# NikolausDemmel/rootba

Measured on NVIDIA B200. Metric: ms/LM-iter (linearize+QR+PCG) on BAL at 1/2/4/8 B200 vs CPU ref, lower is better.
Workload: dtype f32

## Files before the change

rootba_b200/csrc/kernels.cuh:

```cuda
#pragma once

#include <cooperative_groups.h>
#include <cuda_runtime.h>

#include <cfloat>
#include <cmath>
#include <cstdint>

#include "layout.hpp"

namespace rba {

template <class S> struct ST;
template <> struct ST<float> {
  using V2 = float2;
  using V4 = float4;
  __host__ __device__ static float eps_sqrt() { return 0.0031622776601683794f; }
  __host__ __device__ static float eps() { return 1e-5f; }
  __host__ __device__ static float tiny() { return FLT_MIN; }
};
template <> struct ST<double> {
  using V2 = double2;
  using V4 = double4;
  __host__ __device__ static double eps_sqrt() { return 1e-5; }
// ... 1401 lines not shown
  for (int c = lane; c < CP; c += 32) {
    S v = 0;
    if (c < ncols) {
      const int i = c / 9, p = c - 9 * i;
      v = xvec[9 * (size_t)D.slot_cam[T.slot_base + i] + p];
    }
    xs[c] = v;
    ys[c] = 0;
  }
  __syncwarp();
  const V2* __restrict__ prow = reinterpret_cast<const V2*>(D.panel + T.panel_off) + (size_t)it.row0 * KP * 32 + lane;
  for (int r = 0; r < it.nrows; ++r) {
    S d = 0;
    for (int k = 0; k < KP; ++k) {
      const V2 v = __ldg(prow + (size_t)(r * KP + k) * 32);
      const int c = 2 * lane + 64 * k;
      d += v.x * xs[c] + v.y * xs[c + 1];
    }
    d = warp_sum(d);
    for (int k = 0; k < KP; ++k) {
      const V2 v = __ldg(prow + (size_t)(r * KP + k) * 32);
      const int c = 2 * lane + 64 * k;
      ys[c] += d * v.x;
      ys[c + 1] += d * v.y;
    }
  }
  __syncwarp();
  for (int c = lane; c < ncols; c += 32) D.yobs[9 * (size_t)it.yslot_base + c] = ys[c];
  __syncwarp();
}

__device__ __forceinline__ uint32_t smem_u32(const void* p) { return (uint32_t)__cvta_generic_to_shared(p); }
__device__ __forceinline__ void mbar_init(uint64_t* bar, uint32_t count) {
  asm volatile("mbarrier.init.shared::cta.b64 [%0], %1;" ::"r"(smem_u32(bar)), "r"(count) : "memory");
}
__device__ __forceinline__ void mbar_fence_init() {
  asm volatile("fence.mbarrier_init.release.cluster;" ::: "memory");
  asm volatile("fence.proxy.async.shared::cta;" ::: "memory");
}
__device__ __forceinline__ void mbar_expect_tx(uint64_t* bar, uint32_t bytes) {
  asm volatile("mbarrier.arrive.expect_tx.shared::cta.b64 _, [%0], %1;" ::"r"(smem_u32(bar)), "r"(bytes) : "memory");
}
__device__ __forceinline__ uint64_t l2_evict_first_policy() {
  uint64_t pol;
  asm volatile("createpolicy.fractional.L2::evict_first.b64 %0, 1.0;" : "=l"(pol));
  return pol;
}
__device__ __forceinline__ void bulk_g2s(void* dst, const void* src, uint32_t bytes, uint64_t* bar, uint64_t policy) {
  asm volatile("cp.async.bulk.shared::cluster.global.mbarrier::complete_tx::bytes.L2::cache_hint [%0], [%1], %2, [%3], %4;" ::"r"(
                   smem_u32(dst)),
               "l"(src), "r"(bytes), "r"(smem_u32(bar)), "l"(policy)
               : "memory");
}
__device__ __forceinline__ void mbar_wait(uint64_t* bar, uint32_t parity) {
  uint32_t ok;
  const uint32_t a = smem_u32(bar);
  do {
    asm volatile("{\n .reg .pred p;\n mbarrier.try_wait.parity.shared::cta.b64 p, [%1], %2;\n selp.u32 %0, 1, 0, p;\n}"
                 : "=r"(ok)
                 : "r"(a), "r"(parity)
                 : "memory");
  } while (!ok);
}

template <class S>
struct PanelStream {
  const S* src;
  int rows_left;
  int row_scalars;
  int rows_per_stage;
  int next_item;
  unsigned issued;
  uint64_t policy;
};

template <class S, int NS, int STAGE_BYTES>
__device__ __forceinline__ bool stream_produce(PanelStream<S>& ps, const DevPtrs<S>& D, const MatvecItem* __restrict__ items,
                                               int item_end, int item_stride, unsigned char* ring, uint64_t* bars, int lane) {
  if (ps.rows_left == 0) {
    if (ps.next_item >= item_end) return false;
    const MatvecItem it = items[ps.next_item];
    if (it.nrows == 0) { ps.next_item = item_end; return false; }
    const TileInfo T = D.tiles[it.tile];
    ps.row_scalars = T.KP * 64;
    ps.src = D.panel + T.panel_off + (size_t)it.row0 * ps.row_scalars;
    ps.rows_left = it.nrows;
    ps.rows_per_stage = max(1, STAGE_BYTES / (int)(ps.row_scalars * sizeof(S)));
    ps.next_item += item_stride;
  }
  const int rows = min(ps.rows_per_stage, ps.rows_left);
  const uint32_t bytes = (uint32_t)(rows * ps.row_scalars * sizeof(S));
  const unsigned slot = ps.issued % NS;
  if (lane == 0) {
    mbar_expect_tx(&bars[slot], bytes);
    bulk_g2s(ring + (size_t)slot * STAGE_BYTES, ps.src, bytes, &bars[slot], ps.policy);
  }
  ps.src += (size_t)rows * ps.row_scalars;
  ps.rows_left -= rows;
  ++ps.issued;
  return true;
}

template <class T>
__device__ __forceinline__ T group_sum_p(T v, int G) {
  T t;
  t = __shfl_xor_sync(0xffffffffu, v, 16); if (G > 16) v += t;
  t = __shfl_xor_sync(0xffffffffu, v, 8);  if (G > 8) v += t;
  t = __shfl_xor_sync(0xffffffffu, v, 4);  if (G > 4) v += t;
  t = __shfl_xor_sync(0xffffffffu, v, 2);  if (G > 2) v += t;
  t = __shfl_xor_sync(0xffffffffu, v, 1);  if (G > 1) v += t;
  return v;
}

template <class S, int KP, int NS, int STAGE_BYTES>
__device__ __forceinline__ void matvec_item_tma(const DevPtrs<S>& D, const MatvecItem& it, const TileInfo& T, int lane,
                                                const S* __restrict__ xvec, PanelStream<S>& ps, unsigned& consumed,
                                                const MatvecItem* __restrict__ items, int item_end, int item_stride,
                                                unsigned char* ring, uint64_t* bars) {
  using V2 = typename ST<S>::V2;
  const int n = T.n, G = T.G;
  const int g = lane / G, j = lane - g * G;
  const int ncols = 9 * n;
  const bool active = g < T.nvalid;
  const int slot0 = T.slot_base + g * n;
  int off0[KP], off1[KP];
  {
    const int step = 2 * G;
    const int di = step / 9, dp = step - 9 * di;
    int c = 2 * j;
    int i = c / 9, p = c - 9 * i;
#pragma unroll
    for (int k = 0; k < KP; ++k) {
      const bool v0 = active && c < ncols, v1 = active && (c + 1) < ncols;
      const int i1 = (p == 8) ? i + 1 : i, p1 = (p == 8) ? 0 : p + 1;
      const int cam0 = v0 ? __ldg(D.slot_cam + slot0 + i) : 0;
      const int cam1 = v1 ? __ldg(D.slot_cam + slot0 + i1) : 0;
      off0[k] = v0 ? 9 * cam0 + p : -1;
      off1[k] = v1 ? 9 * cam1 + p1 : -1;
      c += step; i += di; p += dp;
      if (p >= 9) { p -= 9; ++i; }
    }
  }
  V2 xv[KP], yv[KP];
#pragma unroll
  for (int k = 0; k < KP; ++k) {
    xv[k] = mk2(off0[k] >= 0 ? __ldg(xvec + off0[k]) : S(0), off1[k] >= 0 ? __ldg(xvec + off1[k]) : S(0));
    yv[k] = mk2(S(0), S(0));
  }
  int rows_left = it.nrows;
  constexpr int RPS = (STAGE_BYTES / (int)(KP * 64 * sizeof(S))) > 0 ? (STAGE_BYTES / (int)(KP * 64 * sizeof(S))) : 1;
  while (rows_left > 0) {
    const unsigned slot = consumed % NS;
    mbar_wait(&bars[slot], (consumed / NS) & 1u);
    const int rows = min(RPS, rows_left);
    const V2* st = reinterpret_cast<const V2*>(ring + (size_t)slot * STAGE_BYTES) + lane;
    int r = 0;
#ifndef RBA_K4_PAIR
#define RBA_K4_PAIR 0
#endif
    for (; RBA_K4_PAIR && r + 2 <= rows; r += 2) {
      V2 va[KP], vb[KP];
#pragma unroll
      for (int k = 0; k < KP; ++k) { va[k] = st[(r * KP + k) * 32]; vb[k] = st[((r + 1) * KP + k) * 32]; }
      S da0 = 0, da1 = 0, db0 = 0, db1 = 0;
#pragma unroll
      for (int k = 0; k < KP; ++k) {
        da0 = fma(va[k].x, xv[k].x, da0); da1 = fma(va[k].y, xv[k].y, da1);
        db0 = fma(vb[k].x, xv[k].x, db0); db1 = fma(vb[k].y, xv[k].y, db1);
      }
      S da = da0 + da1, db = db0 + db1;
      da = group_sum_p(da, G); db = group_sum_p(db, G);
#pragma unroll
      for (int k = 0; k < KP; ++k) {
        yv[k].x = fma(da, va[k].x, yv[k].x); yv[k].y = fma(da, va[k].y, yv[k].y);
        yv[k].x = fma(db, vb[k].x, yv[k].x); yv[k].y = fma(db, vb[k].y, yv[k].y);
      }
    }
    for (; r < rows; ++r) {
      V2 va[KP];
#pragma unroll
      for (int k = 0; k < KP; ++k) va[k] = st[(r * KP + k) * 32];
      S da0 = 0, da1 = 0;
#pragma unroll
      for (int k = 0; k < KP; ++k) { da0 = fma(va[k].x, xv[k].x, da0); da1 = fma(va[k].y, xv[k].y, da1); }
      S da = group_sum_p(da0 + da1, G);
#pragma unroll
      for (int k = 0; k < KP; ++k) { yv[k].x = fma(da, va[k].x, yv[k].x); yv[k].y = fma(da, va[k].y, yv[k].y); }
    }
    __syncwarp();
    ++consumed;
    rows_left -= rows;
    stream_produce<S, NS, STAGE_BYTES>(ps, D, items, item_end, item_stride, ring, bars, lane);
  }
  if (active) {
    S* yo = D.yobs + 9 * (size_t)(it.yslot_base + g * n);
#pragma unroll
    for (int k = 0; k < KP; ++k) {
      const int c = 2 * j + 2 * G * k;
      if (c < ncols) yo[c] = yv[k].x;
      if (c + 1 < ncols) yo[c + 1] = yv[k].y;
    }
  }
}

#ifndef RBA_K4_MINB
#define RBA_K4_MINB (sizeof(S) == 4 ? 5 : 2)
#endif
template <class S, int WARPS, int NS, int STAGE_BYTES>
__global__ void __launch_bounds__(WARPS * 32, RBA_K4_MINB) k_matvec_small_tma(DevPtrs<S> D, const MatvecItem* __restrict__ items,
                                                                  int item_begin, int item_end, int scratch_per_warp,
                                                                  const S* __restrict__ xvec, const int* done, int pdl) {
  extern __shared__ __align__(128) unsigned char smem_tma[];
  __shared__ __align__(8) uint64_t bars_all[WARPS][NS];
  if (done && *reinterpret_cast<const volatile int*>(done)) return;
  const int wib = threadIdx.x >> 5, lane = threadIdx.x & 31;
  unsigned char* ring = smem_tma + (size_t)wib * NS * STAGE_BYTES;
  uint64_t* bars = bars_all[wib];
  if (lane == 0) {
#pragma unroll
    for (int s = 0; s < NS; ++s) mbar_init(&bars[s], 1);
    mbar_fence_init();
  }
  __syncwarp();
  const int stride = gridDim.x * WARPS;
  const int first = item_begin + blockIdx.x * WARPS + wib;
  PanelStream<S> ps;
  ps.src = nullptr; ps.rows_left = 0; ps.row_scalars = 0; ps.rows_per_stage = 1; ps.next_item = first; ps.issued = 0; ps.policy = l2_evict_first_policy();
  unsigned consumed = 0;
#pragma unroll 1
  for (int s = 0; s < NS; ++s)
    if (!stream_produce<S, NS, STAGE_BYTES>(ps, D, items, item_end, stride, ring, bars, lane)) break;
  if (pdl) asm volatile("griddepcontrol.wait;" ::: "memory");
  if (done && *done) {
    for (unsigned s = 0; s < ps.issued; ++s) mbar_wait(&bars[s % NS], (s / NS) & 1u);
    return;
  }
  if (pdl) asm volatile("griddepcontrol.launch_dependents;" ::: "memory");
  for (int q = first; q < item_end; q += stride) {
    const MatvecItem it = items[q];
    if (it.nrows == 0) break;
    const TileInfo T = D.tiles[it.tile];
    switch (T.KP) {
      case 5: matvec_item_tma<S, 5, NS, STAGE_BYTES>(D, it, T, lane, xvec, ps, consumed, items, item_end, stride, ring, bars); break;
      case 6: matvec_item_tma<S, 6, NS, STAGE_BYTES>(D, it, T, lane, xvec, ps, consumed, items, item_end, stride, ring, bars); break;
      case 7: matvec_item_tma<S, 7, NS, STAGE_BYTES>(D, it, T, lane, xvec, ps, consumed, items, item_end, stride, ring, bars); break;
      case 8: matvec_item_tma<S, 8, NS, STAGE_BYTES>(D, it, T, lane, xvec, ps, consumed, items, item_end, stride, ring, bars); break;
      case 9: matvec_item_tma<S, 9, NS, STAGE_BYTES>(D, it, T, lane, xvec, ps, consumed, items, item_end, stride, ring, bars); break;
      default: break;
    }
  }
}

template <class S>
__device__ __forceinline__ void lds_rec28(const S* src, S (&v)[28]) {
  if (sizeof(S) == 4) {
    const float4* s4 = reinterpret_cast<const float4*>(src);
#pragma unroll
    for (int q = 0; q < 7; ++q) { const float4 t = s4[q]; v[4 * q] = t.x; v[4 * q + 1] = t.y; v[4 * q + 2] = t.z; v[4 * q + 3] = t.w; }
  } else {
    const double2* s2 = reinterpret_cast<const double2*>(src);
#pragma unroll
    for (int q = 0; q < 14; ++q) { const double2 t = s2[q]; v[2 * q] = t.x; v[2 * q + 1] = t.y; }
  }
}
template <class S>
__device__ __forceinline__ void lds_rec20(const S* src, S (&v)[20]) {
  if (sizeof(S) == 4) {
    const float4* s4 = reinterpret_cast<const float4*>(src);
#pragma unroll
    for (int q = 0; q < 5; ++q) { const float4 t = s4[q]; v[4 * q] = t.x; v[4 * q + 1] = t.y; v[4 * q + 2] = t.z; v[4 * q + 3] = t.w; }
  } else {
    const double2* s2 = reinterpret_cast<const double2*>(src);
#pragma unroll
    for (int q = 0; q < 10; ++q) { const double2 t = s2[q]; v[2 * q] = t.x; v[2 * q + 1] = t.y; }
  }
}

template <class S, int WARPS, int MAXSLOTS, int NS>
__global__ void __launch_bounds__(WARPS * 32) k_matvec_implicit_tma(DevPtrs<S> D, int tile_end, const S* __restrict__ xvec,
                                                                     const int* done, int pdl, int e0_only = 0) {
  static_assert(MAXSLOTS <= 64, "two observations per lane");
  extern __shared__ __align__(128) unsigned char smem_imp[];
  __shared__ __align__(8) uint64_t bars_all[WARPS][NS];
  if (done && *reinterpret_cast<const volatile int*>(done)) return;
  constexpr int QBYTES = MAXSLOTS * 28 * (int)sizeof(S), JBYTES = MAXSLOTS * 20 * (int)sizeof(S);
  constexpr int STAGE = QBYTES + JBYTES;
  const int wib = threadIdx.x >> 5, lane = threadIdx.x & 31;
  unsigned char* base = smem_imp + (size_t)wib * NS * STAGE;
  uint64_t* bars = bars_all[wib];
  if (lane == 0) {
#pragma unroll
    for (int s = 0; s < NS; ++s) mbar_init(&bars[s], 1);
    mbar_fence_init();
  }
  __syncwarp();
  const uint64_t policy = l2_evict_first_policy();
  const int stride = gridDim.x * WARPS;
  const int first = blockIdx.x * WARPS + wib;
  auto produce = [&](int t, int s) {
    if (lane == 0) {
// ... 667 lines not shown
```

rootba_b200/csrc/layout.hpp:

```cpp
#pragma once

#include <algorithm>
#include <cstdint>
#include <numeric>
#include <string>
#include <vector>

namespace rba {

struct TileInfo {
  long long panel_off;
  int slot_base;
  int lm_base;
  short n;
  short G;
  short KP;
  short nvalid;
};

struct MatvecItem {
  int tile;
  short row0, nrows;
  int yslot_base;
  int pad;
};

struct ReduceItem {
  int cam, begin, end;
};

struct CameraCSR {
  std::vector<int> cam_ptr;
  std::vector<int> slots;
  std::vector<ReduceItem> items;
  std::vector<int> cam_item_ptr;
};

struct Layout {
  int nc = 0;
  int lm_begin = 0, lm_end = 0;
  int nl_local = 0;
  long long nobs_local = 0;
  long long sum_n2 = 0;
  int max_n = 0;
  int kp_max = 0;
  std::vector<int> sorted_lm;
  std::vector<int> sorted_of_lm;
  std::vector<TileInfo> tiles;
  std::vector<int> tile_of_sorted;
  int nslots = 0;
  std::vector<int> slot_cam;
  std::vector<int> slot_lm;
  std::vector<long long> slot_obs;
  long long panel_scalars = 0;
  std::vector<MatvecItem> items;
  int n_items_large = 0;
  int nyslots = 0;
  CameraCSR csr_obs;
  CameraCSR csr_y;
  bool csr_y_is_obs = true;
  std::vector<ReduceItem> pb_items;
  std::vector<int> pb_cam_item_ptr;
  int k1_scratch_per_warp = 0;
  int k4_scratch_per_warp = 0;
};

constexpr int KP_SMALL_MAX = 9;
constexpr int ROWS_PER_ITEM = 32;
#ifndef RBA_SEG_LEN
#define RBA_SEG_LEN 96
#endif
constexpr int SEG_LEN = RBA_SEG_LEN;
constexpr int PB_SEG_LEN = 16;

inline int group_size_for(int n) {
  if (n <= 2) return 1;
  if (n <= 4) return 2;
// ... 77 lines not shown
  long long panel = 0;
  size_t pos = 0;
  while (pos < order.size()) {
    const int n = nloc[order[pos]];
    size_t end = pos;
    while (end < order.size() && nloc[order[end]] == n) ++end;
    const int G = group_size_for(n), W = 32 / G, KP = kp_for(n, G);
    for (size_t p = pos; p < end; p += W) {
      TileInfo T;
      T.panel_off = panel;
      T.slot_base = slot;
      T.lm_base = (int)L.sorted_lm.size();
      T.n = (short)n; T.G = (short)G; T.KP = (short)KP;
      T.nvalid = (short)std::min<size_t>(W, end - p);
      for (int g = 0; g < W; ++g) {
        const bool real = g < T.nvalid;
        const int lm = real ? order[p + g] : -1;
        if (real) L.sorted_of_lm[lm] = (int)L.sorted_lm.size();
        L.sorted_lm.push_back(lm);
        L.tile_of_sorted.push_back((int)L.tiles.size());
        for (int i = 0; i < n; ++i) {
          if (real) {
            const int64_t o = lm_off[L.lm_begin + lm] + i;
            L.slot_cam.push_back(obs_cam[o]);
            L.slot_lm.push_back(lm);
            L.slot_obs.push_back(o);
          } else {
            L.slot_cam.push_back(0);
            L.slot_lm.push_back(-1);
            L.slot_obs.push_back(-1);
          }
        }
      }
      slot += W * n;
      panel += (long long)2 * n * KP * 64;
      L.tiles.push_back(T);
    }
    pos = end;
  }
  L.nslots = slot;
  L.panel_scalars = panel;
  int extra = L.nslots;
  std::vector<int> ycam(L.slot_cam.size());
  for (int s = 0; s < L.nslots; ++s) ycam[s] = L.slot_lm[s] >= 0 ? L.slot_cam[s] : -1;
  for (int t = 0; t < (int)L.tiles.size(); ++t) {
    const TileInfo& T = L.tiles[t];
    const int rows = 2 * T.n, W = 32 / T.G;
    int nchunks = 1;
    if (rows > ROWS_PER_ITEM + ROWS_PER_ITEM / 2) nchunks = (rows + ROWS_PER_ITEM - 1) / ROWS_PER_ITEM;
    int r0 = 0;
    for (int c = 0; c < nchunks; ++c) {
      const int r1 = (int)((long long)rows * (c + 1) / nchunks);
      MatvecItem it;
      it.tile = t; it.row0 = (short)r0; it.nrows = (short)(r1 - r0); it.pad = 0;
      if (c == 0) {
        it.yslot_base = T.slot_base;
      } else {
        it.yslot_base = extra;
        for (int g = 0; g < W; ++g)
          for (int i = 0; i < T.n; ++i) {
            const int s = T.slot_base + g * T.n + i;
            ycam.push_back(L.slot_lm[s] >= 0 ? L.slot_cam[s] : -1);
          }
        extra += W * T.n;
        L.csr_y_is_obs = false;
      }
      L.items.push_back(it);
      r0 = r1;
    }
  }
  L.nyslots = extra;
  auto work = [&](const MatvecItem& it) {
    const TileInfo& T = L.tiles[it.tile];
    return (long long)it.nrows * T.KP;
  };
  std::stable_sort(L.items.begin(), L.items.end(), [&](const MatvecItem& a, const MatvecItem& b) {
    const bool la = L.tiles[a.tile].KP > KP_SMALL_MAX, lb = L.tiles[b.tile].KP > KP_SMALL_MAX;
    if (la != lb) return la;
    return work(a) > work(b);
  });
  L.n_items_large = 0;
  for (auto& it : L.items) if (L.tiles[it.tile].KP > KP_SMALL_MAX) ++L.n_items_large;
  {
    std::vector<int> ocam(ycam.begin(), ycam.begin() + L.nslots);
    build_csr(nc, L.nslots, ocam, L.csr_obs);
    if (!L.csr_y_is_obs) build_csr(nc, L.nyslots, ycam, L.csr_y);
    L.pb_cam_item_ptr.assign(nc + 1, 0);
    for (int c = 0; c < nc; ++c) {
      L.pb_cam_item_ptr[c] = (int)L.pb_items.size();
      for (int b = L.csr_obs.cam_ptr[c]; b < L.csr_obs.cam_ptr[c + 1]; b += PB_SEG_LEN)
        L.pb_items.push_back({c, b, std::min(b + PB_SEG_LEN, L.csr_obs.cam_ptr[c + 1])});
    }
    L.pb_cam_item_ptr[nc] = (int)L.pb_items.size();
  }
  for (const TileInfo& T : L.tiles) {
    const int W = 32 / T.G;
    L.k1_scratch_per_warp = std::max(L.k1_scratch_per_warp, W * 32 * (int)T.n);
    const int CS = (2 * T.G * T.KP) | 1;
    L.k4_scratch_per_warp = std::max(L.k4_scratch_per_warp, T.KP > kp_max ? 2 * 64 * (int)T.KP : W * CS);
  }
  return "";
}

}
```

rootba_b200/csrc/solver.cu:

```cuda
#include <cuda_runtime.h>
#include <dlfcn.h>

#include <cstdio>
#include <cstdlib>
#include <cstring>
#include <chrono>
#include <limits>
#include <memory>
#include <string>
#include <vector>

#include "../../include/rootba_b200.h"
#include "../host/bal_io_fast.hpp"
#include "kernels.cuh"
#include "nccl_dyn.hpp"

namespace rba {

thread_local std::string g_err;

#define CU(call)                                                                                   \
  do {                                                                                             \
    cudaError_t e__ = (call);                                                                      \
    if (e__ != cudaSuccess) {                                                                      \
// ... 11 lines not shown

using namespace rba;

struct rba_handle {
  int scalar_size = 0;
  virtual ~rba_handle() {}
  virtual int set_state(const void* cams, const void* lms) = 0;
  virtual int get_state(void* cams, void* lms) = 0;
  virtual int backup() = 0;
  virtual int restore() = 0;
  virtual int compute_error(rba_residual_info* out) = 0;
  virtual int linearize() = 0;
  virtual int solve(double lambda, void* inc_out, rba_cg_summary* cg) = 0;
  virtual int apply(const void* inc, void* l_diff_out, bool update_cameras) = 0;
  virtual int lm_step(bool linearize_first, double lambda, rba_lm_step_result* out) = 0;
  virtual int lm_run(const rba_lm_opts* o, int max_steps, rba_lm_iteration* log, int* steps_done, int* terminated, rba_stage_timings* totals) = 0;
  virtual int get_timings(rba_stage_timings* out) const = 0;
  virtual int get_stats(rba_workload_stats* out) const = 0;
  virtual int get_scaling(void* scaling, void* diag2) = 0;
  virtual int get_rhs(void* b) = 0;
  virtual int get_precond(void* inv, void* blocks) = 0;
  virtual int right_multiply(const void* x, void* y) = 0;
  virtual int debug_get_block(int lm, void* out, int rows, int cols, void* jls) = 0;
  virtual int time_matvec(int reps, double* sec) = 0;
  virtual int timer_start() = 0;
  virtual int timer_stop(double* sec) = 0;
  virtual void* stream_ptr() = 0;
  virtual int synchronize() = 0;
  virtual int comm_init(const void* uid) = 0;
  virtual int ipc_export(void* out128) = 0;
  virtual int ipc_import(const void* all) = 0;
};

#ifndef RBA_IMP_NS
#define RBA_IMP_NS 1
#endif

namespace rba {

template <class S>
struct Solver : rba_handle {
  rba_solver_opts opt{};
  KOpts ko{};
  Layout L;
  int nc = 0, nl_total = 0;
  int device = 0;
  int sm_count = 148;
  cudaStream_t stream = nullptr;
  std::vector<void*> allocs;
  size_t device_bytes = 0;
  DevPtrs<S> D{};
  S* cams_bk = nullptr; S* lms_bk = nullptr;
  MatvecItem* d_items = nullptr;
  std::vector<MatvecItem> dealt_items;
  int n_dealt = 0, dealt_grid = 0, dealt_bps = 0;
  long long state_version = 0;
  rba_residual_info error_cache{}; long long error_cache_version = -1, error_enqueue_version = -1; bool error_cache_valid = false;
  int* d_csr_obs_slots = nullptr; ReduceItem* d_csr_obs_items = nullptr; int* d_csr_obs_item_ptr = nullptr;
  int* d_csr_y_slots = nullptr; ReduceItem* d_csr_y_items = nullptr; int* d_csr_y_item_ptr = nullptr;
  int n_obs_items = 0, n_y_items = 0;
  const int* op_slots = nullptr; const ReduceItem* op_items = nullptr; const int* op_item_ptr = nullptr; int n_op_items = 0;
  bool implicit_op = false;
  int e0_only_flag = 0;
  bool panel_form = true;
  int imp_tile_split = 0;
  size_t imp_smem = 0; int imp_grid = 1;
  ReduceItem* d_pb_items = nullptr; int* d_pb_item_ptr = nullptr; int n_pb_items = 0;
  int pcg_cluster = 16;
  bool use_pdl = true;
  int* h_prog = nullptr; int* d_prog = nullptr;
  int pcg_solve_id = 0;
  bool pcg_partials = true;
  double* d_epart = nullptr;
  double* d_red = nullptr;
  int* d_flags = nullptr;
  int* d_cam_cnt = nullptr;
  PcgState* d_state = nullptr;
  PcgState* h_state = nullptr;
  double* h_red = nullptr;
  int* h_flags = nullptr;
  cudaEvent_t poll_ev[2] = {nullptr, nullptr};
  bool linearized = false;
  bool new_linearization_point = false;
  bool have_inc = false;
  S last_lambda = 0;
  bool damping_valid = false;
  rba_stage_timings tm{};
  EventPair ev_stage1, ev_stage2, ev_precond, ev_pcg, ev_backsub, ev_update, ev_error, ev_mv, ev_user;
  long long launches = 0;
  NcclApi* nccl = nullptr;
  ncclComm_t comm = nullptr;
  char* peer_mem = nullptr;
  size_t peer_bytes = 0;
  PeerComm pc{};
  bool peer_ok = false;
  int ar_seq = 0, c_seq = 0, s_seq = 0;
  std::vector<void*> ipc_opened;
  static constexpr int EBLOCKS = 592;
  static constexpr int KPMAX = sizeof(S) == 4 ? 16 : 10;

  ~Solver() override {
    if (comm && nccl) nccl->CommDestroy(comm);
    for (void* p : ipc_opened) cudaIpcCloseMemHandle(p);
    for (void* p : allocs) cudaFree(p);
    if (h_prog) cudaFreeHost(h_prog);
    if (h_state) cudaFreeHost(h_state);
// ... 61 lines not shown
    ko.use_valid_projections_only = opt.use_valid_projections_only;
    ko.robust_norm = opt.robust_norm;
    ko.write_panel = (opt.operator_form == 1 || opt.solver_type != 0) ? 0 : 1;
    ko.huber = opt.huber_parameter;
    ko.jacobi_eps = opt.jacobi_scaling_epsilon > 0 ? opt.jacobi_scaling_epsilon : (double)ST<S>::eps_sqrt();
    std::string msg = build_layout(nc, nl_total, pv->lm_obs_offset, pv->obs_cam_idx, opt.rank, opt.nranks, KPMAX, L);
    if (!msg.empty()) { g_err = msg; return RBA_ERR_INVALID_ARGUMENT; }
    std::vector<S> xy((size_t)2 * L.nslots, S(0));
    const S* src = (const S*)pv->obs_xy;
    for (int s = 0; s < L.nslots; ++s)
      if (L.slot_obs[s] >= 0) { xy[2 * (size_t)s] = src[2 * L.slot_obs[s]]; xy[2 * (size_t)s + 1] = src[2 * L.slot_obs[s] + 1]; }
    int rc;
    TileInfo* d_tiles; int* d_sorted; int* d_slot_cam; int* d_slot_lm; S* d_xy;
#define TRY(x) do { rc = (x); if (rc) return rc; } while (0)
    TRY(upload(&d_tiles, L.tiles));
    TRY(upload(&d_sorted, L.sorted_lm));
    TRY(upload(&d_slot_cam, L.slot_cam));
    TRY(upload(&d_slot_lm, L.slot_lm));
    TRY(upload(&d_xy, xy));
    dealt_items = L.items;
    n_dealt = (int)L.items.size();
    {
      const char* e = getenv("RBA_MATVEC_DEAL");
      long long deal_ovh = 48;
      if (const char* o2 = getenv("RBA_MATVEC_DEAL_OVH")) deal_ovh = atoll(o2);
      const int nsmall = (int)L.items.size() - L.n_items_large;
      int tma_bps = std::max(1, (int)((220 * 1024) / ((size_t)K4_WARPS * K4_NS * K4_STAGE + 1024)));
      {
        const size_t smem = (size_t)K4_WARPS * K4_NS * K4_STAGE;
        int occ = 0;
        if (cudaFuncSetAttribute((k_matvec_small_tma<S, K4_WARPS, K4_NS, K4_STAGE>), cudaFuncAttributeMaxDynamicSharedMemorySize, (int)smem) == cudaSuccess &&
            cudaOccupancyMaxActiveBlocksPerMultiprocessor(&occ, (k_matvec_small_tma<S, K4_WARPS, K4_NS, K4_STAGE>), K4_WARPS * 32, smem) == cudaSuccess && occ > 0)
          tma_bps = std::min(tma_bps, occ);
        else
          cudaGetLastError();
      }
      dealt_bps = tma_bps;
      const int W = grid_for(nsmall, K4_WARPS, tma_bps) * K4_WARPS;
      if (!(e && std::string(e) == "rr") && nsmall > W && !implicit_op) {
        std::vector<std::vector<int>> lists(W);
        std::vector<std::pair<long long, int>> heap(W);
        for (int w = 0; w < W; ++w) heap[w] = {0, w};
        auto cmp = [](const std::pair<long long, int>& a, const std::pair<long long, int>& b) { return a > b; };
        std::make_heap(heap.begin(), heap.end(), cmp);
        for (int q = L.n_items_large; q < (int)L.items.size(); ++q) {
          std::pop_heap(heap.begin(), heap.end(), cmp);
          auto& top = heap.back();
          lists[top.second].push_back(q);
          top.first += (long long)L.items[q].nrows * L.tiles[L.items[q].tile].KP + deal_ovh;
          std::push_heap(heap.begin(), heap.end(), cmp);
        }
        size_t maxlen = 0;
        for (auto& l : lists) maxlen = std::max(maxlen, l.size());
        MatvecItem empty{}; empty.tile = 0; empty.row0 = 0; empty.nrows = 0; empty.yslot_base = 0; empty.pad = 0;
        dealt_items.assign(L.items.begin(), L.items.begin() + L.n_items_large);
        dealt_items.resize(L.n_items_large + maxlen * W, empty);
        for (int w = 0; w < W; ++w)
          for (size_t k = 0; k < lists[w].size(); ++k) dealt_items[L.n_items_large + k * W + w] = L.items[lists[w][k]];
        n_dealt = (int)dealt_items.size();
        dealt_grid = W / K4_WARPS;
      }
    }
    TRY(upload(&d_items, dealt_items));

    TRY(upload(&d_csr_obs_slots, L.csr_obs.slots));
    TRY(upload(&d_csr_obs_items, L.csr_obs.items));
    TRY(upload(&d_csr_obs_item_ptr, L.csr_obs.cam_item_ptr));
    n_obs_items = (int)L.csr_obs.items.size();
    if (L.csr_y_is_obs) {
      d_csr_y_slots = d_csr_obs_slots; d_csr_y_items = d_csr_obs_items; d_csr_y_item_ptr = d_csr_obs_item_ptr;
      n_y_items = n_obs_items;
    } else {
      TRY(upload(&d_csr_y_slots, L.csr_y.slots));
      TRY(upload(&d_csr_y_items, L.csr_y.items));
      TRY(upload(&d_csr_y_item_ptr, L.csr_y.cam_item_ptr));
      n_y_items = (int)L.csr_y.items.size();
    }
    implicit_op = opt.operator_form == 1 || opt.solver_type != 0;
    if (opt.operator_form != 0 && opt.operator_form != 1) { g_err = "operator_form must be 0 (dense) or 1 (implicit)"; return RBA_ERR_INVALID_ARGUMENT; }
    if (opt.solver_type < 0 || opt.solver_type > 2) { g_err = "solver_type must be 0 (SQUARE_ROOT), 1 (SCHUR_COMPLEMENT) or 2 (POWER_SCHUR_COMPLEMENT)"; return RBA_ERR_INVALID_ARGUMENT; }
    if (opt.solver_type == 2 && opt.nranks > 1) { g_err = "POWER_SCHUR_COMPLEMENT runs on one GPU (the power-series vector kernel has no peer exchange yet)"; return RBA_ERR_UNSUPPORTED; }
    if (opt.power_order <= 0) opt.power_order = 20;
    if (opt.solver_type != 0) implicit_op = true;
    if (opt.stage2_form != 0 && opt.stage2_form != 1) { g_err = "stage2_form must be 0 (Q2 panel, reference) or 1 (orthogonality identity)"; return RBA_ERR_INVALID_ARGUMENT; }
    panel_form = !implicit_op && opt.stage2_form == 0;
    if (implicit_op) {
      while (imp_tile_split < (int)L.tiles.size() && (32 / L.tiles[imp_tile_split].G) * L.tiles[imp_tile_split].n <= IMP_MAXSLOTS) ++imp_tile_split;
      imp_smem = (size_t)IMP_WARPS * IMP_NS * (size_t)IMP_MAXSLOTS * 48 * sizeof(S);
      CU(cudaFuncSetAttribute((k_matvec_implicit_tma<S, IMP_WARPS, IMP_MAXSLOTS, IMP_NS>), cudaFuncAttributeMaxDynamicSharedMemorySize, (int)imp_smem));
      int bps = 0;
      CU(cudaOccupancyMaxActiveBlocksPerMultiprocessor(&bps, (k_matvec_implicit_tma<S, IMP_WARPS, IMP_MAXSLOTS, IMP_NS>), IMP_WARPS * 32, imp_smem));
      imp_grid = std::max(1, std::min((imp_tile_split + IMP_WARPS - 1) / IMP_WARPS, sm_count * std::max(1, bps)));
    }
    if (implicit_op) { op_slots = d_csr_obs_slots; op_items = d_csr_obs_items; op_item_ptr = d_csr_obs_item_ptr; n_op_items = n_obs_items; }
    else { op_slots = d_csr_y_slots; op_items = d_csr_y_items; op_item_ptr = d_csr_y_item_ptr; n_op_items = n_y_items; }
    TRY(upload(&d_pb_items, L.pb_items));
    TRY(upload(&d_pb_item_ptr, L.pb_cam_item_ptr));
    n_pb_items = (int)L.pb_items.size();
    D.tiles = d_tiles; D.ntiles = (int)L.tiles.size(); D.sorted_lm = d_sorted;
    D.slot_cam = d_slot_cam; D.slot_lm = d_slot_lm; D.slot_xy = d_xy; D.nslots = L.nslots; D.nc = nc;
    TRY(dalloc(&D.cams, (size_t)10 * nc)); TRY(dalloc(&cams_bk, (size_t)10 * nc));
    TRY(dalloc(&D.lms, (size_t)3 * L.nl_local)); TRY(dalloc(&lms_bk, (size_t)3 * L.nl_local));
    if (ko.write_panel) TRY(dalloc(&D.panel, (size_t)L.panel_scalars));
    TRY(dalloc(&D.jp, (size_t)20 * L.nslots));
    TRY(dalloc(&D.q1u, (size_t)28 * L.nslots));
    TRY(dalloc(&D.q1d, (size_t)28 * L.nslots));
    TRY(dalloc(&D.jl, (size_t)6 * L.nslots));
    TRY(dalloc(&D.res, (size_t)2 * L.nslots));
    TRY(dalloc(&D.lmk, (size_t)24 * L.sorted_lm.size()));
    TRY(dalloc(&D.qtr, (size_t)2 * L.nslots));
    if (panel_form) {
      TRY(dalloc(&D.dmp, (size_t)28 * L.nslots));
      if (opt.preconditioner_type == 1) TRY(dalloc(&D.blk0, (size_t)48 * L.nslots));
      TRY(dalloc(&D.blocks0, (size_t)81 * nc));
// ... 48 lines not shown
      };
      TRY(setup(k1_sc, K1_CAP, need1, k1_smem, k1_bps, k1_max_blocks));
      TRY(setup(k2_sc, K2_CAP, need2, k2_smem, k2_bps, k2_max_blocks));
      if (!(getenv("RBA_TILE_DEAL") && std::string(getenv("RBA_TILE_DEAL")) == "rr")) {
        TRY(deal_tiles(tile_grid(k1_max_blocks) * TILE_WARPS, order_k1));
        TRY(deal_tiles(tile_grid(sm_count * 8) * TILE_WARPS, order_kp));
      }
      CU(cudaFuncSetAttribute((k_linearize_qr<S, false>), cudaFuncAttributeMaxDynamicSharedMemorySize, (int)k1_smem));
      CU(cudaFuncSetAttribute((k_linearize_qr<S, true>), cudaFuncAttributeMaxDynamicSharedMemorySize, (int)k1_smem));
      CU(cudaFuncSetAttribute((k_stage2<S, true>), cudaFuncAttributeMaxDynamicSharedMemorySize, (int)k2_smem));
      CU(cudaFuncSetAttribute((k_stage2<S, false>), cudaFuncAttributeMaxDynamicSharedMemorySize, (int)k2_smem));
    }
    k4_smem_small = (size_t)K4_WARPS * L.k4_scratch_per_warp * sizeof(S);
    if (k4_smem_small > 200 * 1024) { g_err = "matvec scratch exceeds shared memory"; return RBA_ERR_UNSUPPORTED; }
    CU(cudaFuncSetAttribute(k_matvec_small<S, K4_WARPS>, cudaFuncAttributeMaxDynamicSharedMemorySize, (int)std::max<size_t>(k4_smem_small, 1024)));
    CU(cudaFuncSetAttribute((k_matvec_large<S, K4_WARPS, KPMAX>), cudaFuncAttributeMaxDynamicSharedMemorySize, (int)std::max<size_t>(k4_smem_small, 1024)));
    {
      CU(cudaFuncSetAttribute(k_pcg_vec<S>, cudaFuncAttributeNonPortableClusterSizeAllowed, 1));
      CU(cudaFuncSetAttribute(k_power_vec<S>, cudaFuncAttributeNonPortableClusterSizeAllowed, 1));
      pcg_cluster = 16;
      if (const char* e = getenv("RBA_PDL")) use_pdl = atoi(e) != 0;
      if (const char* e = getenv("RBA_PCG_PARTIALS")) pcg_partials = atoi(e) != 0;
      if (const char* e = getenv("RBA_PCG_CLUSTER")) pcg_cluster = std::max(1, std::min(atoi(e), 16));
      for (; pcg_cluster > 1; pcg_cluster >>= 1) {
        cudaLaunchConfig_t cfg = {};
        cfg.gridDim = dim3(pcg_cluster); cfg.blockDim = dim3(VEC_THREADS);
        cudaLaunchAttribute at[1];
        at[0].id = cudaLaunchAttributeClusterDimension;
        at[0].val.clusterDim.x = pcg_cluster; at[0].val.clusterDim.y = 1; at[0].val.clusterDim.z = 1;
        cfg.attrs = at; cfg.numAttrs = 1;
        int ncl = 0;
        if (cudaOccupancyMaxActiveClusters(&ncl, k_pcg_vec<S>, &cfg) == cudaSuccess && ncl >= 1) break;
        cudaGetLastError();
      }
    }
    {
      const char* e = getenv("RBA_MATVEC");
      use_tma = !(e && std::string(e) == "ldg");
      k4_smem_tma = (size_t)K4_WARPS * K4_NS * K4_STAGE;
      if (k4_smem_tma > 220 * 1024) use_tma = false;
      if (use_tma) {
        CU(cudaFuncSetAttribute((k_matvec_small_tma<S, K4_WARPS, K4_NS, K4_STAGE>), cudaFuncAttributeMaxDynamicSharedMemorySize, (int)k4_smem_tma));
        k4_tma_blocks_per_sm = std::max(1, (int)((220 * 1024) / (k4_smem_tma + 1024)));
        if (dealt_bps > 0) k4_tma_blocks_per_sm = dealt_bps;
        if (const char* b = getenv("RBA_MATVEC_BLOCKS_PER_SM")) k4_tma_blocks_per_sm = std::max(1, atoi(b));
      }
    }
#undef TRY
    CU(cudaStreamSynchronize(stream));
    return RBA_OK;
  }
  static constexpr int K4_WARPS = 4;
  static constexpr int IMP_WARPS = 2, IMP_MAXSLOTS = 64, IMP_NS = RBA_IMP_NS;
#ifndef RBA_K4_NS
#define RBA_K4_NS 2
#endif
#ifndef RBA_K4_STAGE
#define RBA_K4_STAGE 4608
#endif
  static constexpr int K4_NS = RBA_K4_NS;
  static constexpr int K4_STAGE = RBA_K4_STAGE;
  static constexpr int TILE_WARPS = 4;
  static constexpr int K1_CAP = 3904;
  static constexpr int K2_CAP = 3072;
  Scratch<S> k1_sc{}, k2_sc{};
  size_t k1_smem = 0, k2_smem = 0;
  int k1_bps = 2, k2_bps = 2, k1_max_blocks = 296, k2_max_blocks = 296;
  size_t k4_smem_small = 0, k4_smem_tma = 0;
  bool use_tma = true;
  int k4_tma_blocks_per_sm = 2;

  int allreduce(S* buf, size_t count) {
    if (opt.nranks == 1) return RBA_OK;
    if (peer_ok && (long long)count <= pc.cmax) {
      ++c_seq;
      const int g = (int)std::max<size_t>(1, std::min<size_t>((size_t)sm_count, (count + 255) / 256));
      k_peer_push<S><<<g, 256, 0, stream>>>(pc, buf, (long long)count, c_seq & 1);
      k_peer_sum<S><<<g, 256, 0, stream>>>(pc, buf, (long long)count, c_seq & 1, c_seq, d_flags + 1);
      launches += 2;
      return RBA_OK;
    }
    if (!comm) { g_err = "rba_comm_init has not been called on a sharded handle"; return RBA_ERR_STATE; }
    ncclResult_t r = nccl->AllReduce(buf, buf, count, sizeof(S) == 4 ? ncclFloat : ncclDouble, ncclSum, comm, stream);
    if (r != ncclSuccess) { g_err = std::string("ncclAllReduce: ") + nccl->GetErrorString(r); return RBA_ERR_NCCL; }
    return RBA_OK;
  }
  int allreduce_scalars(int nd) {
    if (opt.nranks == 1) return RBA_OK;
    if (peer_ok) {
      ++s_seq;
      k_peer_small<<<1, 64, 0, stream>>>(pc, d_red, nd, d_flags, 4, s_seq & 1, s_seq, d_flags + 1);
      ++launches;
      return RBA_OK;
    }
    if (!comm) { g_err = "rba_comm_init has not been called on a sharded handle"; return RBA_ERR_STATE; }
    ncclResult_t r = ncclSuccess;
    if (nd > 0) r = nccl->AllReduce(d_red, d_red, nd, ncclDouble, ncclSum, comm, stream);
    if (r == ncclSuccess) r = nccl->AllReduce(d_flags, d_flags, 4, ncclInt, ncclSum, comm, stream);
    if (r != ncclSuccess) { g_err = std::string("ncclAllReduce: ") + nccl->GetErrorString(r); return RBA_ERR_NCCL; }
    return RBA_OK;
  }

  int comm_init(const void* uid) override {
    if (opt.nranks == 1) return RBA_OK;
    nccl = nccl_api();
    if (!nccl) { g_err = "libnccl.so.2 could not be loaded"; return RBA_ERR_NCCL; }
    ncclUniqueId id;
    std::memcpy(&id, uid, sizeof(id));
    CU(cudaSetDevice(device));
    ncclResult_t r = nccl->CommInitRank(&comm, opt.nranks, id, opt.rank);
    if (r != ncclSuccess) { g_err = std::string("ncclCommInitRank: ") + nccl->GetErrorString(r); return RBA_ERR_NCCL; }
    return RBA_OK;
  }

// ... 190 lines not shown
    CU(cudaGetLastError());
    tm.stage1_time = elapsed(ev_stage1);
    tm.kernel_launches = launches - lin_l0;
    if (h_flags[4 + 1]) { linearized = false; g_err = "a peer rank did not take part in a cross-shard reduction in time (peer-memory exchange timed out)"; return RBA_ERR_NCCL; }
    if (h_flags[4 + 0]) { linearized = false; return RBA_NUMERICAL_FAILURE; }
    return RBA_OK;
  }
  int linearize() override {
    int rc = linearize_enqueue(); if (rc) return rc;
    CU(cudaStreamSynchronize(stream));
    return linearize_finish();
  }

  int precond_blocks(int mode, S* dst, const S* addend, bool reduce_ranks) {
    const int g = (n_pb_items + 127) / 128;
    switch (mode) {
      case 0: k_precond_partial<S, 0><<<g, 128, 0, stream>>>(D.jp, (const S*)nullptr, d_csr_obs_slots, d_pb_items, n_pb_items, D.pblk); break;
      case 1: k_precond_partial<S, 1><<<g, 128, 0, stream>>>(D.jp, D.q1d, d_csr_obs_slots, d_pb_items, n_pb_items, D.pblk); break;
      case 2: k_precond_partial<S, 2><<<g, 128, 0, stream>>>(D.dmp, (const S*)nullptr, d_csr_obs_slots, d_pb_items, n_pb_items, D.pblk); break;
      default: k_precond_partial<S, 3><<<g, 128, 0, stream>>>(D.blk0, (const S*)nullptr, d_csr_obs_slots, d_pb_items, n_pb_items, D.pblk); break;
    }
    k_precond_final<S><<<(45 * nc + 255) / 256, 256, 0, stream>>>(D.pblk, d_pb_item_ptr, nc, addend, dst);
    launches += 2;
    return reduce_ranks ? allreduce(dst, (size_t)81 * nc) : RBA_OK;
  }

  void matvec_launch(const S* xvec, const int* done) {
    matvec_kernels(xvec, done);
    k_cam_reduce_final<S, false><<<grid_for(n_op_items, 8, 8), 256, 0, stream>>>((const S*)D.yobs, op_slots, op_items, n_op_items, op_item_ptr, D.partial,
                                                                               d_cam_cnt, D.y, done, 0, pc, 0, nc);
    ++launches;
  }
  void matvec_kernels(const S* xvec, const int* done, bool pdl = false) {
    if (implicit_op) {
      const int ntl = (int)L.tiles.size();
      const bool p = pdl && use_pdl && imp_tile_split == ntl;
      if (imp_tile_split > 0 && use_tma)
        launch_ex((k_matvec_implicit_tma<S, IMP_WARPS, IMP_MAXSLOTS, IMP_NS>), imp_grid, IMP_WARPS * 32, imp_smem, p, 1, D, imp_tile_split, xvec, done, (int)p, e0_only_flag);
      const int tb = use_tma ? imp_tile_split : 0;
      if (tb < ntl)
        launch_ex(k_matvec_implicit<S>, (ntl - tb + TILE_WARPS - 1) / TILE_WARPS, TILE_WARPS * 32, 0, false, 1, D, tb, xvec, done, 0, e0_only_flag);
      ++tm.matvec_launches;
      return;
    }
    const int nitems = n_dealt;
    if (L.n_items_large > 0) {
      k_matvec_large<S, K4_WARPS, KPMAX><<<grid_for(L.n_items_large, K4_WARPS, 4), K4_WARPS * 32, k4_smem_small, stream>>>(
          D, d_items, 0, L.n_items_large, L.k4_scratch_per_warp, xvec, done);
      ++launches;
    }
    if (nitems > L.n_items_large) {
      if (use_tma) {
        launch_ex(k_matvec_small_tma<S, K4_WARPS, K4_NS, K4_STAGE>, dealt_grid > 0 ? dealt_grid : grid_for(nitems - L.n_items_large, K4_WARPS, k4_tma_blocks_per_sm), K4_WARPS * 32,
                  k4_smem_tma, pdl && use_pdl && L.n_items_large == 0, 1, D, (const MatvecItem*)d_items, L.n_items_large, nitems, L.k4_scratch_per_warp, xvec, done,
                  (int)(pdl && use_pdl && L.n_items_large == 0));
        --launches;
      } else
        k_matvec_small<S, K4_WARPS><<<grid_for(nitems - L.n_items_large, K4_WARPS, 5), K4_WARPS * 32, k4_smem_small, stream>>>(
            D, d_items, L.n_items_large, nitems, L.k4_scratch_per_warp, xvec, done);
      ++launches;
    }
    ++tm.matvec_launches;
  }
  int pcg_vec(int i, int mode, bool pdl, int is_last, S lambda, bool fused_ar = false, bool from_partials = false) {
    PeerComm c = pc;
    if (!fused_ar) c.nranks = 1;
    return launch_ex(k_pcg_vec<S>, pcg_cluster, VEC_THREADS, 0, pdl && use_pdl, pcg_cluster, D, d_state, lambda, i, mode, (double)opt.eta,
                     (int)opt.min_linear_solver_iterations, is_last, (int)(pdl && use_pdl), c, ar_seq, from_partials ? op_item_ptr : (const int*)nullptr, d_prog);
  }
  bool pcg_from_partials() const {
    return opt.nranks == 1 && pcg_partials && 9 * ((nc + pcg_cluster - 1) / pcg_cluster) <= VEC_THREADS * VEC_EPT;
  }
  int pcg_apply(int i, int mode, int is_last, S lambda) {
    if (pcg_from_partials()) {
      int rc = launch_ex(k_cam_reduce<S>, grid_for(n_op_items, 8, 8), 256, 0, use_pdl, 1, (const S*)D.yobs, op_slots, op_items, n_op_items, D.partial,
                         (const int*)&d_state->done, (int)use_pdl);
      if (rc) return rc;
      return pcg_vec(i, mode, true, is_last, lambda, false, true);
    }
    const bool fused = opt.nranks > 1 && peer_ok;
    if (fused) ++ar_seq;
    if (opt.nranks > 1 && !fused) CU(cudaMemsetAsync(D.y, 0, (size_t)9 * nc * sizeof(S), stream));
    int rc = fused ? launch_ex((k_cam_reduce_final<S, true>), grid_for(n_op_items, 8, 8), 256, 0, use_pdl, 1, (const S*)D.yobs, op_slots,
                               op_items, n_op_items, op_item_ptr, D.partial, d_cam_cnt, D.y, (const int*)&d_state->done, (int)use_pdl, pc, ar_seq, nc)
                   : launch_ex((k_cam_reduce_final<S, false>), grid_for(n_op_items, 8, 8), 256, 0, use_pdl, 1, (const S*)D.yobs, op_slots,
                               op_items, n_op_items, op_item_ptr, D.partial, d_cam_cnt, D.y, (const int*)&d_state->done, (int)use_pdl, pc, ar_seq, nc);
    if (rc) return rc;
    if (opt.nranks == 1) return pcg_vec(i, mode, true, is_last, lambda);
    if (fused) return pcg_vec(i, mode, true, is_last, lambda, true);
    rc = allreduce(D.y, (size_t)9 * nc); if (rc) return rc;
    return pcg_vec(i, mode, false, is_last, lambda);
  }
  int matvec_finish(const S* vec, S* out, S lambda, PcgState* st, double* part) {
    int rc = allreduce(D.y, (size_t)9 * nc); if (rc) return rc;
    k_pcg_q<S><<<NPART, 128, 0, stream>>>(D, st, nullptr, nullptr, D.y, vec, out, lambda, part);
    ++launches;
    return RBA_OK;
  }

  int power_enqueue(void* inc_out) {
    int rc = start(ev_pcg); if (rc) return rc;
    CU(cudaMemsetAsync(d_state, 0, sizeof(PcgState), stream));
    const int order = opt.power_order, chk = opt.pcg_check_period;
    rc = launch_ex(k_power_vec<S>, pcg_cluster, VEC_THREADS, 0, false, pcg_cluster, D, d_state, 0, (double)opt.eta, 0, 0); if (rc) return rc;
    e0_only_flag = 1;
    int i = 1, pending[2] = {0, 0}, slot = 0;
    bool finished = false;
// ... 637 lines not shown
```

Before: 8.977.

## Prefetch per-item camera offsets and headers via TMA alongside panel stream

Packs each small matvec item's tile metadata (n, G, KP, nvalid, yslot, nrows) and precomputed 9*camera offsets into a per-item run in a new global array. This run is bulk-copied into shared memory on the same mbarrier as the panel stage. The consumer then reads item headers and x offsets from shared memory instead of doing dependent global loads of items, tiles and slot_cam. It also replaces the predicated shuffle reduction with a switch-based fallthrough and removes the unused paired-row path and compile-time knobs. The cost is extra static shared memory per warp and a larger host-side preprocessing step.

```diff
diff --git a/rootba_b200/csrc/kernels.cuh b/rootba_b200/csrc/kernels.cuh
--- a/rootba_b200/csrc/kernels.cuh
+++ b/rootba_b200/csrc/kernels.cuh
@@ -1477,6 +1477,11 @@
                "l"(src), "r"(bytes), "r"(smem_u32(bar)), "l"(policy)
                : "memory");
 }
+__device__ __forceinline__ void bulk_g2s(void* dst, const void* src, uint32_t bytes, uint64_t* bar) {
+  asm volatile("cp.async.bulk.shared::cluster.global.mbarrier::complete_tx::bytes [%0], [%1], %2, [%3];" ::"r"(smem_u32(dst)),
+               "l"(src), "r"(bytes), "r"(smem_u32(bar))
+               : "memory");
+}
 __device__ __forceinline__ void mbar_wait(uint64_t* bar, uint32_t parity) {
   uint32_t ok;
   const uint32_t a = smem_u32(bar);
@@ -1488,6 +1493,8 @@
   } while (!ok);
 }
 
+constexpr int K4_RUN_HDR = 4;
+constexpr int K4_RUN_MAX = K4_RUN_HDR + 64;
 template <class S>
 struct PanelStream {
   const S* src;
@@ -1496,12 +1503,16 @@
   int rows_per_stage;
   int next_item;
   unsigned issued;
+  unsigned opened;
   uint64_t policy;
 };
 
 template <class S, int NS, int STAGE_BYTES>
 __device__ __forceinline__ bool stream_produce(PanelStream<S>& ps, const DevPtrs<S>& D, const MatvecItem* __restrict__ items,
-                                               int item_end, int item_stride, unsigned char* ring, uint64_t* bars, int lane) {
+                                               const int* __restrict__ xoff, int item_end, int item_stride, unsigned char* ring,
+                                               uint64_t* bars, int* xbuf, int lane) {
+  uint32_t xbytes = 0;
+  const int* xsrc = nullptr;
   if (ps.rows_left == 0) {
     if (ps.next_item >= item_end) return false;
     const MatvecItem it = items[ps.next_item];
@@ -1512,14 +1523,18 @@
     ps.rows_left = it.nrows;
     ps.rows_per_stage = max(1, STAGE_BYTES / (int)(ps.row_scalars * sizeof(S)));
     ps.next_item += item_stride;
+    xsrc = xoff + it.xoff;
+    xbytes = (uint32_t)((K4_RUN_HDR + ((T.nvalid * T.n + 3) & ~3)) * sizeof(int));
   }
   const int rows = min(ps.rows_per_stage, ps.rows_left);
   const uint32_t bytes = (uint32_t)(rows * ps.row_scalars * sizeof(S));
   const unsigned slot = ps.issued % NS;
   if (lane == 0) {
-    mbar_expect_tx(&bars[slot], bytes);
+    mbar_expect_tx(&bars[slot], bytes + xbytes);
+    if (xbytes) bulk_g2s(xbuf + (ps.opened % NS) * K4_RUN_MAX, xsrc, xbytes, &bars[slot]);
     bulk_g2s(ring + (size_t)slot * STAGE_BYTES, ps.src, bytes, &bars[slot], ps.policy);
   }
+  if (xbytes) ++ps.opened;
   ps.src += (size_t)rows * ps.row_scalars;
   ps.rows_left -= rows;
   ++ps.issued;
@@ -1536,18 +1551,30 @@
   t = __shfl_xor_sync(0xffffffffu, v, 1);  if (G > 1) v += t;
   return v;
 }
+template <class T>
+__device__ __forceinline__ T group_sum_j(T v, int G) {
+  switch (G) {
+    case 32: v += __shfl_xor_sync(0xffffffffu, v, 16); [[fallthrough]];
+    case 16: v += __shfl_xor_sync(0xffffffffu, v, 8); [[fallthrough]];
+    case 8: v += __shfl_xor_sync(0xffffffffu, v, 4); [[fallthrough]];
+    case 4: v += __shfl_xor_sync(0xffffffffu, v, 2); [[fallthrough]];
+    case 2: v += __shfl_xor_sync(0xffffffffu, v, 1); [[fallthrough]];
+    default: break;
+  }
+  return v;
+}
 
 template <class S, int KP, int NS, int STAGE_BYTES>
-__device__ __forceinline__ void matvec_item_tma(const DevPtrs<S>& D, const MatvecItem& it, const TileInfo& T, int lane,
-                                                const S* __restrict__ xvec, PanelStream<S>& ps, unsigned& consumed,
-                                                const MatvecItem* __restrict__ items, int item_end, int item_stride,
-                                                unsigned char* ring, uint64_t* bars) {
+__device__ __forceinline__ void matvec_item_tma(const DevPtrs<S>& D, int n, int G, int nvalid, int nrows, int yslot_base,
+                                                const int* xo, int lane, const S* __restrict__ xvec, PanelStream<S>& ps,
+                                                unsigned& consumed, const MatvecItem* __restrict__ items,
+                                                const int* __restrict__ xoff, int item_end, int item_stride,
+                                                unsigned char* ring, uint64_t* bars, int* xbuf) {
   using V2 = typename ST<S>::V2;
-  const int n = T.n, G = T.G;
   const int g = lane / G, j = lane - g * G;
   const int ncols = 9 * n;
-  const bool active = g < T.nvalid;
-  const int slot0 = T.slot_base + g * n;
+  const bool active = g < nvalid;
+  xo += g * n;
   int off0[KP], off1[KP];
   {
     const int step = 2 * G;
@@ -1558,10 +1585,8 @@
     for (int k = 0; k < KP; ++k) {
       const bool v0 = active && c < ncols, v1 = active && (c + 1) < ncols;
       const int i1 = (p == 8) ? i + 1 : i, p1 = (p == 8) ? 0 : p + 1;
-      const int cam0 = v0 ? __ldg(D.slot_cam + slot0 + i) : 0;
-      const int cam1 = v1 ? __ldg(D.slot_cam + slot0 + i1) : 0;
-      off0[k] = v0 ? 9 * cam0 + p : -1;
-      off1[k] = v1 ? 9 * cam1 + p1 : -1;
+      off0[k] = v0 ? xo[i] + p : -1;
+      off1[k] = v1 ? xo[i1] + p1 : -1;
       c += step; i += di; p += dp;
       if (p >= 9) { p -= 9; ++i; }
     }
@@ -1572,53 +1597,31 @@
     xv[k] = mk2(off0[k] >= 0 ? __ldg(xvec + off0[k]) : S(0), off1[k] >= 0 ? __ldg(xvec + off1[k]) : S(0));
     yv[k] = mk2(S(0), S(0));
   }
-  int rows_left = it.nrows;
+  int rows_left = nrows;
   constexpr int RPS = (STAGE_BYTES / (int)(KP * 64 * sizeof(S))) > 0 ? (STAGE_BYTES / (int)(KP * 64 * sizeof(S))) : 1;
   while (rows_left > 0) {
     const unsigned slot = consumed % NS;
     mbar_wait(&bars[slot], (consumed / NS) & 1u);
     const int rows = min(RPS, rows_left);
     const V2* st = reinterpret_cast<const V2*>(ring + (size_t)slot * STAGE_BYTES) + lane;
-    int r = 0;
-#ifndef RBA_K4_PAIR
-#define RBA_K4_PAIR 0
-#endif
-    for (; RBA_K4_PAIR && r + 2 <= rows; r += 2) {
-      V2 va[KP], vb[KP];
-#pragma unroll
-      for (int k = 0; k < KP; ++k) { va[k] = st[(r * KP + k) * 32]; vb[k] = st[((r + 1) * KP + k) * 32]; }
-      S da0 = 0, da1 = 0, db0 = 0, db1 = 0;
-#pragma unroll
-      for (int k = 0; k < KP; ++k) {
-        da0 = fma(va[k].x, xv[k].x, da0); da1 = fma(va[k].y, xv[k].y, da1);
-        db0 = fma(vb[k].x, xv[k].x, db0); db1 = fma(vb[k].y, xv[k].y, db1);
-      }
-      S da = da0 + da1, db = db0 + db1;
-      da = group_sum_p(da, G); db = group_sum_p(db, G);
-#pragma unroll
-      for (int k = 0; k < KP; ++k) {
-        yv[k].x = fma(da, va[k].x, yv[k].x); yv[k].y = fma(da, va[k].y, yv[k].y);
-        yv[k].x = fma(db, vb[k].x, yv[k].x); yv[k].y = fma(db, vb[k].y, yv[k].y);
-      }
-    }
-    for (; r < rows; ++r) {
+    for (int r = 0; r < rows; ++r) {
       V2 va[KP];
 #pragma unroll
       for (int k = 0; k < KP; ++k) va[k] = st[(r * KP + k) * 32];
       S da0 = 0, da1 = 0;
 #pragma unroll
       for (int k = 0; k < KP; ++k) { da0 = fma(va[k].x, xv[k].x, da0); da1 = fma(va[k].y, xv[k].y, da1); }
-      S da = group_sum_p(da0 + da1, G);
+      S da = group_sum_j(da0 + da1, G);
 #pragma unroll
       for (int k = 0; k < KP; ++k) { yv[k].x = fma(da, va[k].x, yv[k].x); yv[k].y = fma(da, va[k].y, yv[k].y); }
     }
     __syncwarp();
     ++consumed;
     rows_left -= rows;
-    stream_produce<S, NS, STAGE_BYTES>(ps, D, items, item_end, item_stride, ring, bars, lane);
+    stream_produce<S, NS, STAGE_BYTES>(ps, D, items, xoff, item_end, item_stride, ring, bars, xbuf, lane);
   }
   if (active) {
-    S* yo = D.yobs + 9 * (size_t)(it.yslot_base + g * n);
+    S* yo = D.yobs + 9 * (size_t)(yslot_base + g * n);
 #pragma unroll
     for (int k = 0; k < KP; ++k) {
       const int c = 2 * j + 2 * G * k;
@@ -1628,19 +1631,18 @@
   }
 }
 
-#ifndef RBA_K4_MINB
-#define RBA_K4_MINB (sizeof(S) == 4 ? 5 : 2)
-#endif
 template <class S, int WARPS, int NS, int STAGE_BYTES>
-__global__ void __launch_bounds__(WARPS * 32, RBA_K4_MINB) k_matvec_small_tma(DevPtrs<S> D, const MatvecItem* __restrict__ items,
-                                                                  int item_begin, int item_end, int scratch_per_warp,
+__global__ void __launch_bounds__(WARPS * 32, sizeof(S) == 4 ? 5 : 2) k_matvec_small_tma(DevPtrs<S> D, const MatvecItem* __restrict__ items,
+                                                                  const int* __restrict__ xoff, int item_begin, int item_end,
                                                                   const S* __restrict__ xvec, const int* done, int pdl) {
   extern __shared__ __align__(128) unsigned char smem_tma[];
   __shared__ __align__(8) uint64_t bars_all[WARPS][NS];
+  __shared__ __align__(16) int xbuf_all[WARPS][NS * K4_RUN_MAX];
   if (done && *reinterpret_cast<const volatile int*>(done)) return;
   const int wib = threadIdx.x >> 5, lane = threadIdx.x & 31;
   unsigned char* ring = smem_tma + (size_t)wib * NS * STAGE_BYTES;
   uint64_t* bars = bars_all[wib];
+  int* xbuf = xbuf_all[wib];
   if (lane == 0) {
 #pragma unroll
     for (int s = 0; s < NS; ++s) mbar_init(&bars[s], 1);
@@ -1650,27 +1652,29 @@
   const int stride = gridDim.x * WARPS;
   const int first = item_begin + blockIdx.x * WARPS + wib;
   PanelStream<S> ps;
-  ps.src = nullptr; ps.rows_left = 0; ps.row_scalars = 0; ps.rows_per_stage = 1; ps.next_item = first; ps.issued = 0; ps.policy = l2_evict_first_policy();
-  unsigned consumed = 0;
+  ps.src = nullptr; ps.rows_left = 0; ps.row_scalars = 0; ps.rows_per_stage = 1; ps.next_item = first; ps.issued = 0; ps.opened = 0;
+  ps.policy = l2_evict_first_policy();
+  unsigned consumed = 0, nitem = 0;
 #pragma unroll 1
   for (int s = 0; s < NS; ++s)
-    if (!stream_produce<S, NS, STAGE_BYTES>(ps, D, items, item_end, stride, ring, bars, lane)) break;
+    if (!stream_produce<S, NS, STAGE_BYTES>(ps, D, items, xoff, item_end, stride, ring, bars, xbuf, lane)) break;
   if (pdl) asm volatile("griddepcontrol.wait;" ::: "memory");
   if (done && *done) {
     for (unsigned s = 0; s < ps.issued; ++s) mbar_wait(&bars[s % NS], (s / NS) & 1u);
     return;
   }
   if (pdl) asm volatile("griddepcontrol.launch_dependents;" ::: "memory");
-  for (int q = first; q < item_end; q += stride) {
-    const MatvecItem it = items[q];
-    if (it.nrows == 0) break;
-    const TileInfo T = D.tiles[it.tile];
-    switch (T.KP) {
-      case 5: matvec_item_tma<S, 5, NS, STAGE_BYTES>(D, it, T, lane, xvec, ps, consumed, items, item_end, stride, ring, bars); break;
-      case 6: matvec_item_tma<S, 6, NS, STAGE_BYTES>(D, it, T, lane, xvec, ps, consumed, items, item_end, stride, ring, bars); break;
-      case 7: matvec_item_tma<S, 7, NS, STAGE_BYTES>(D, it, T, lane, xvec, ps, consumed, items, item_end, stride, ring, bars); break;
-      case 8: matvec_item_tma<S, 8, NS, STAGE_BYTES>(D, it, T, lane, xvec, ps, consumed, items, item_end, stride, ring, bars); break;
-      case 9: matvec_item_tma<S, 9, NS, STAGE_BYTES>(D, it, T, lane, xvec, ps, consumed, items, item_end, stride, ring, bars); break;
+  while (nitem != ps.opened) {
+    const int* run = xbuf + (nitem++ % NS) * K4_RUN_MAX;
+    mbar_wait(&bars[consumed % NS], (consumed / NS) & 1u);
+    const int4 h = *reinterpret_cast<const int4*>(run);
+    const int n = h.x & 0xffff, G = h.x >> 16, nvalid = h.y >> 16;
+    switch (h.y & 0xffff) {
+      case 5: matvec_item_tma<S, 5, NS, STAGE_BYTES>(D, n, G, nvalid, h.w, h.z, run + K4_RUN_HDR, lane, xvec, ps, consumed, items, xoff, item_end, stride, ring, bars, xbuf); break;
+      case 6: matvec_item_tma<S, 6, NS, STAGE_BYTES>(D, n, G, nvalid, h.w, h.z, run + K4_RUN_HDR, lane, xvec, ps, consumed, items, xoff, item_end, stride, ring, bars, xbuf); break;
+      case 7: matvec_item_tma<S, 7, NS, STAGE_BYTES>(D, n, G, nvalid, h.w, h.z, run + K4_RUN_HDR, lane, xvec, ps, consumed, items, xoff, item_end, stride, ring, bars, xbuf); break;
+      case 8: matvec_item_tma<S, 8, NS, STAGE_BYTES>(D, n, G, nvalid, h.w, h.z, run + K4_RUN_HDR, lane, xvec, ps, consumed, items, xoff, item_end, stride, ring, bars, xbuf); break;
+      case 9: matvec_item_tma<S, 9, NS, STAGE_BYTES>(D, n, G, nvalid, h.w, h.z, run + K4_RUN_HDR, lane, xvec, ps, consumed, items, xoff, item_end, stride, ring, bars, xbuf); break;
       default: break;
     }
   }
diff --git a/rootba_b200/csrc/layout.hpp b/rootba_b200/csrc/layout.hpp
--- a/rootba_b200/csrc/layout.hpp
+++ b/rootba_b200/csrc/layout.hpp
@@ -22,7 +22,7 @@
   int tile;
   short row0, nrows;
   int yslot_base;
-  int pad;
+  int xoff;
 };
 
 struct ReduceItem {
@@ -206,7 +206,7 @@
     for (int c = 0; c < nchunks; ++c) {
       const int r1 = (int)((long long)rows * (c + 1) / nchunks);
       MatvecItem it;
-      it.tile = t; it.row0 = (short)r0; it.nrows = (short)(r1 - r0); it.pad = 0;
+      it.tile = t; it.row0 = (short)r0; it.nrows = (short)(r1 - r0); it.xoff = 0;
       if (c == 0) {
         it.yslot_base = T.slot_base;
       } else {
diff --git a/rootba_b200/csrc/solver.cu b/rootba_b200/csrc/solver.cu
--- a/rootba_b200/csrc/solver.cu
+++ b/rootba_b200/csrc/solver.cu
@@ -87,6 +87,7 @@
   DevPtrs<S> D{};
   S* cams_bk = nullptr; S* lms_bk = nullptr;
   MatvecItem* d_items = nullptr;
+  int* d_item_xoff = nullptr;
   std::vector<MatvecItem> dealt_items;
   int n_dealt = 0, dealt_grid = 0, dealt_bps = 0;
   long long state_version = 0;
@@ -254,7 +255,7 @@
         }
         size_t maxlen = 0;
         for (auto& l : lists) maxlen = std::max(maxlen, l.size());
-        MatvecItem empty{}; empty.tile = 0; empty.row0 = 0; empty.nrows = 0; empty.yslot_base = 0; empty.pad = 0;
+        MatvecItem empty{}; empty.tile = 0; empty.row0 = 0; empty.nrows = 0; empty.yslot_base = 0; empty.xoff = 0;
         dealt_items.assign(L.items.begin(), L.items.begin() + L.n_items_large);
         dealt_items.resize(L.n_items_large + maxlen * W, empty);
         for (int w = 0; w < W; ++w)
@@ -262,6 +263,20 @@
         n_dealt = (int)dealt_items.size();
         dealt_grid = W / K4_WARPS;
       }
+    }
+    {
+      std::vector<int> xoff;
+      for (int q = L.n_items_large; q < n_dealt; ++q) {
+        MatvecItem& it = dealt_items[q];
+        if (it.nrows == 0) continue;
+        const TileInfo& T = L.tiles[it.tile];
+        it.xoff = (int)xoff.size();
+        xoff.insert(xoff.end(), {T.n | (T.G << 16), T.KP | (T.nvalid << 16), it.yslot_base, it.nrows});
+        for (int s = 0; s < T.nvalid * T.n; ++s) xoff.push_back(9 * L.slot_cam[T.slot_base + s]);
+        xoff.resize((xoff.size() + 3) & ~(size_t)3, 0);
+      }
+      if (xoff.empty()) xoff.assign(4, 0);
+      TRY(upload(&d_item_xoff, xoff));
     }
     TRY(upload(&d_items, dealt_items));
 
@@ -416,14 +431,8 @@
   }
   static constexpr int K4_WARPS = 4;
   static constexpr int IMP_WARPS = 2, IMP_MAXSLOTS = 64, IMP_NS = RBA_IMP_NS;
-#ifndef RBA_K4_NS
-#define RBA_K4_NS 2
-#endif
-#ifndef RBA_K4_STAGE
-#define RBA_K4_STAGE 4608
-#endif
-  static constexpr int K4_NS = RBA_K4_NS;
-  static constexpr int K4_STAGE = RBA_K4_STAGE;
+  static constexpr int K4_NS = 2;
+  static constexpr int K4_STAGE = 4608;
   static constexpr int TILE_WARPS = 4;
   static constexpr int K1_CAP = 3904;
   static constexpr int K2_CAP = 3072;
@@ -720,7 +729,7 @@
     if (nitems > L.n_items_large) {
       if (use_tma) {
         launch_ex(k_matvec_small_tma<S, K4_WARPS, K4_NS, K4_STAGE>, dealt_grid > 0 ? dealt_grid : grid_for(nitems - L.n_items_large, K4_WARPS, k4_tma_blocks_per_sm), K4_WARPS * 32,
-                  k4_smem_tma, pdl && use_pdl && L.n_items_large == 0, 1, D, (const MatvecItem*)d_items, L.n_items_large, nitems, L.k4_scratch_per_warp, xvec, done,
+                  k4_smem_tma, pdl && use_pdl && L.n_items_large == 0, 1, D, (const MatvecItem*)d_items, (const int*)d_item_xoff, L.n_items_large, nitems, xvec, done,
                   (int)(pdl && use_pdl && L.n_items_large == 0));
         --launches;
       } else
```

Result: slower. 9.339 (median of 6 runs) (+4.0%).
